# hpc4cmb/flacarray

Hardware: AMD Instinct MI355X
Metric: Msamples/s encode+decode, 4096ch x 1Msamp int32 (higher is better)
Workload: dtype int32

## Files before the change

### flacarray_amd/csrc/encode_fused.hpp

```cpp
#pragma once
#include "encode_kernels.hpp"
#include "quantize_kernels.hpp"

namespace fa {

constexpr int kFSmpWords = 65 * 32;
#ifndef FA_F_SCANW
#define FA_F_SCANW 4
#endif
#ifndef FA_F_RING
#define FA_F_RING 1024
#endif
constexpr int kFRingWords = FA_F_RING;
constexpr int kFRingMask = kFRingWords - 1;
constexpr int kFRingBlocks = kFRingWords / 64;
constexpr int kFRowBlocks = 12;
static_assert(kFRingBlocks - kFRowBlocks - 1 >= 1, "the ring must hold the longest row and a partial block beside what waits to be flushed");
constexpr int kFWaveWords = kFSmpWords + kFRingWords + 4 + 16;
constexpr int kFWaves = 4;
constexpr int kFCrcSlice = 1024;
constexpr int kFCrcXpow = 520;
#ifndef FA_F_SLEEP
#define FA_F_SLEEP 8
#endif
#ifndef FA_F_WBATCH
#define FA_F_WBATCH 4
#endif
#ifndef FA_F_CEIL
#define FA_F_CEIL 1
#endif
#ifndef FA_F_BFLY_N
#define FA_F_BFLY_N 1
#endif
#ifndef FA_F_SHLEV
#define FA_F_SHLEV 1
#endif
#ifndef FA_F_SHLEV_MAXMLO
#define FA_F_SHLEV_MAXMLO 12
#endif
#ifndef FA_F_SHPOLL
#define FA_F_SHPOLL 256
#endif
#ifndef FA_F_SHSLEEP
#define FA_F_SHSLEEP 4
#endif
#ifndef FA_F_PARKN
#define FA_F_PARKN 32
#endif
#ifndef FA_F_PARKBLK
#define FA_F_PARKBLK 1
#endif
#ifndef FA_F_PARK
#define FA_F_PARK 1
#endif
#ifndef FA_F_WAVES
#define FA_F_WAVES 3
#endif
constexpr uint32_t kLbSpinLimit = 1u << 22;

struct FusedArgs {
    const int32_t* data;
    const float* f_offsets;
    const float* f_gains;
    int64_t n_stream, stream_size, nframes, total_frames;
    int32_t max_lpc_order, max_porder, precision, pmax_full;
    int32_t tail_bs;
    double escale_full;
    const float* win;
    const uint4* hdr;
    uint8_t* blob;
    int64_t capacity;
    int64_t hb;
    uint32_t* frame_bytes;
    int64_t* frame_abs;
    FrameInfo* info;
    uint32_t* ticket;
    uint32_t* size_pub;
    unsigned long long* off_pub;
    int64_t* total;
    int* err;
    const uint16_t* crc_tab;
    unsigned long long* stamps;
    int64_t* starts;
    int64_t* nbytes;
};

__device__ __forceinline__ int fsmp_unit(int c1, int u) { return 32 * c1 + 4 * (u ^ (c1 & 7)); }
__device__ __forceinline__ int fsmp_idx(int s) {
    const int c1 = (s >> 5) + 1;
    return fsmp_unit(c1, (s >> 2) & 7) + (s & 3);
}

__device__ __forceinline__ int lane_id_opaque() {
    int l;
    asm volatile("v_mbcnt_lo_u32_b32 %0, -1, 0\n\tv_mbcnt_hi_u32_b32 %0, -1, %0" : "=v"(l));
    return l;
}
__device__ __forceinline__ int rice_fold(int r) { return (int)(((uint32_t)r << 1) ^ (uint32_t)(r >> 31)); }
__device__ __forceinline__ int dpp_wave_shr1(int old, int v) { return __builtin_amdgcn_update_dpp(old, v, 0x138, 0xF, 0xF, false); }

__device__ __forceinline__ uint16_t crc16_mulmod(uint16_t a, uint16_t b) {
    uint32_t r = 0;
#pragma unroll
    for (int i = 15; i >= 0; --i) {
        r = (r << 1) ^ ((r & 0x8000u) ? 0x18005u : 0u);
        if ((b >> i) & 1) r ^= a;
    }
    return (uint16_t)r;
}

template <typename T>
__device__ __forceinline__ T lb_load(const T* p) { return __hip_atomic_load(p, __ATOMIC_RELAXED, __HIP_MEMORY_SCOPE_AGENT); }

struct SplitRiceSearch {
    int pred_order, pmax, lane;
    uint32_t TA, TB, S, n, pb, SC, best;
    int M, p, k, bpo, kb;
    bool slot;
    __device__ __forceinline__ void start(uint32_t ta, uint32_t tb, int pred_order_, int pmax_, int lane_) {
        pred_order = pred_order_; pmax = pmax_; lane = lane_;
        TA = wave_incl_scan_u32(ta);
        TB = wave_incl_scan_u32(tb);
    }
    __device__ __forceinline__ void gather() {
        M = (2 << pmax) - 1;
        const int Lp = M - lane;
        slot = (Lp >= 1);
        const int po = slot ? (31 - __clz(Lp)) : 0;
        p = lane - (M + 1 - (2 << po));
        const uint32_t psz = 4096u >> po;
        const int cpp = 128 >> po;
        const bool inB = (po > 0) && (p >= (1 << (po - 1)));
        const int ph = inB ? (p - (1 << (po - 1))) : p;
        int hi_l = (po == 0) ? 63 : ((ph + 1) * cpp - 1);
        int lo_l = (po == 0) ? -1 : (ph * cpp - 1);
        hi_l &= 63;
        const int lo_c = lo_l < 0 ? 0 : (lo_l & 63);
        const uint32_t ah = (uint32_t)__builtin_amdgcn_ds_bpermute(hi_l << 2, (int)TA);
        const uint32_t bh = (uint32_t)__builtin_amdgcn_ds_bpermute(hi_l << 2, (int)TB);
        const uint32_t al = (uint32_t)__builtin_amdgcn_ds_bpermute(lo_c << 2, (int)TA);
        const uint32_t bl = (uint32_t)__builtin_amdgcn_ds_bpermute(lo_c << 2, (int)TB);
        uint32_t s;
        if (po == 0) s = ah + bh;
        else s = (inB ? bh : ah) - ((lo_l >= 0) ? (inB ? bl : al) : 0u);
        S = slot ? s : 0u;
        n = psz - ((p == 0) ? (uint32_t)pred_order : 0u);
        n = slot ? n : 1u;
    }
    __device__ __forceinline__ void params() {
        const uint32_t fpd = 0x40000u / n;
        const uint32_t m1 = S - 1;
// ... 188 lines not shown
                }
            } else {
                double* mbv = reinterpret_cast<double*>(wscr + 224);
                if (sub < MLO) mbv[sub] = mybits;
                lds_fence();
#pragma unroll
                for (int o = 0; o < MLO; ++o) {
                    const double b = mbv[o];
                    if (o < usable && b < bestb) { bestb = b; bi = o; }
                }
            }
            wlo = bi + 1;
        }
        if (fbps <= 17) {
            const int limp = 32 - fbps - ilog2_u64((uint64_t)wlo);
            if (wprec > limp) wprec = limp;
        }
        wsh = 0;
#pragma unroll
        for (int j = 0; j < MLO; ++j) wq[j] = 0;
        wok = 0;
        if (wprec >= 2) wok = (quantize_coefs_t<MLO>(coef + (wlo - 1) * MLO, wlo, wprec, wq, &wsh) == 0) ? 1 : 0;
    };
    auto shlev_announce = [&](bool cand, int fbps, const double* ac) __attribute__((always_inline)) {
        const int ln = lane_id_opaque();
        if (ln == 0) {
            if (cand) {
#pragma unroll
                for (int j = 0; j <= MLO; ++j) lev_in[wave][j] = ac[j];
            }
            lev_bps[wave] = cand ? fbps : -1;
        }
        lds_fence();
        uint32_t before = 0;
        if (ln == 0) before = __hip_atomic_fetch_add(&lev_cnt, 1u, __ATOMIC_RELAXED, __HIP_MEMORY_SCOPE_WORKGROUP);
        lds_fence();
        if ((uint32_t)__builtin_amdgcn_readfirstlane((int)before) != (uint32_t)(kFWaves - 1)) return;
        const int fr = ln >> 4, sub = ln & 15;
        const int fbps_w = lev_bps[fr];
        double acw[MLO + 1];
#pragma unroll
        for (int j = 0; j <= MLO; ++j) acw[j] = lev_in[fr][j];
        if (fbps_w < 0) {
            acw[0] = 1.0;
#pragma unroll
            for (int j = 1; j <= MLO; ++j) acw[j] = 0.0;
        }
        int wok, wlo, wprec, wsh;
        int32_t wq[MLO];
        lpc_solve(std::integral_constant<int, 16>{}, acw, fbps_w, scr + 256 * fr, sub, wok, wlo, wprec, wsh, wq);
        if (sub == 0) {
            lev_out[fr][0] = wok; lev_out[fr][1] = wlo; lev_out[fr][2] = wprec; lev_out[fr][3] = wsh;
#pragma unroll
            for (int j = 0; j < MLO; ++j) lev_out[fr][4 + j] = wq[j];
        }
        lds_fence();
        if (sub == 0) __hip_atomic_store(&lev_rdy[fr], 1u, __ATOMIC_RELAXED, __HIP_MEMORY_SCOPE_WORKGROUP);
        lds_fence();
    };
    if constexpr (SHLEV) {
        bool mine = g < a.total_frames;
        if (mine && a.tail_bs != kMaxBlock) mine = ((uint32_t)g % (uint32_t)a.nframes) != (uint32_t)(a.nframes - 1);
        if (__builtin_expect(!mine, 0)) {
            shlev_announce(false, 0, nullptr);
            return;
        }
    }
    if (g >= a.total_frames) return;

    const int64_t s = (int64_t)((uint32_t)g / (uint32_t)a.nframes);
    const int64_t f = g - s * a.nframes;
    if (f == a.nframes - 1 && a.tail_bs != kMaxBlock) return;
    const int32_t* src = a.data + (s * a.stream_size + f * (int64_t)bs);
    float q_off = 0.0f, q_gain = 0.0f;
    if constexpr (F32IN) { q_off = a.f_offsets[s]; q_gain = a.f_gains[s]; }
    auto load_row = [&](int j) __attribute__((always_inline)) {
        const int4 v = reinterpret_cast<const int4*>(src)[64 * j + lane];
        if constexpr (F32IN)
            return make_int4(quantise_f32(__int_as_float(v.x), q_off, q_gain), quantise_f32(__int_as_float(v.y), q_off, q_gain),
                             quantise_f32(__int_as_float(v.z), q_off, q_gain), quantise_f32(__int_as_float(v.w), q_off, q_gain));
        else
            return v;
    };
    const float* win = a.win;
    const uint4 fhe = a.hdr[f];
    const uint32_t fh_bits = 32u + ((fhe.w >> 8) & 0xFFu) + ((fhe.w >> 16) & 0xFFu) + (fhe.w >> 24) + 8u;

#define FA_IMAGE_ADDRS                                                                  \
    const int ln_ = lane_id_opaque();                                                   \
    const int K = fsmp_unit(ln_ + 1, 0);                                                \
    const int rowbase = fsmp_unit((ln_ >> 3) + 1, ln_ & 7);                             \
    const int hist7 = fsmp_unit(ln_, 7), hist6 = fsmp_unit(ln_, 6), hist5 = fsmp_unit(ln_, 5); \
    (void)K; (void)rowbase; (void)hist7; (void)hist6; (void)hist5
    constexpr int tailA7 = 32 * 64 + 4 * (7 ^ (64 & 7)), tailA6 = 32 * 64 + 4 * (6 ^ (64 & 7)), tailA5 = 32 * 64 + 4 * (5 ^ (64 & 7));

    FA_STAMP_INIT;
#ifdef FA_TIMELINE
    const uint32_t tl_start_ = (uint32_t)__builtin_amdgcn_s_memrealtime();
#endif
    int4 Bv[8];
    uint32_t orv = 0;
    int mn, mx;
    {
        FA_IMAGE_ADDRS;
        int4 hi[8], lo[8];
#pragma unroll
        for (int j = 0; j < 8; ++j) hi[j] = load_row(8 + j);
#pragma unroll
        for (int j = 0; j < 8; ++j) lo[j] = load_row(j);
        if (lane < 32) smp[lane] = 0;
        mn = hi[0].x;
        mx = hi[0].x;
#pragma unroll
        for (int j = 0; j < 8; ++j) {
            orv |= (uint32_t)(hi[j].x | hi[j].y | hi[j].z | hi[j].w);
            mn = min(min(mn, hi[j].x), hi[j].y);
            mn = min(min(mn, hi[j].z), hi[j].w);
            mx = max(max(mx, hi[j].x), hi[j].y);
            mx = max(max(mx, hi[j].z), hi[j].w);
            *reinterpret_cast<int4*>(&smp[rowbase + 256 * j]) = hi[j];
        }
#pragma unroll
        for (int t = 0; t < 8; ++t) Bv[t] = *reinterpret_cast<const int4*>(&smp[K ^ (4 * t)]);
#pragma unroll
        for (int j = 0; j < 8; ++j) {
            orv |= (uint32_t)(lo[j].x | lo[j].y | lo[j].z | lo[j].w);
            mn = min(min(mn, lo[j].x), lo[j].y);
            mn = min(min(mn, lo[j].z), lo[j].w);
            mx = max(max(mx, lo[j].x), lo[j].y);
            mx = max(max(mx, lo[j].z), lo[j].w);
            *reinterpret_cast<int4*>(&smp[rowbase + 256 * j]) = lo[j];
        }
    }
    mn = wave_min_i32(mn);
    mx = wave_max_i32(mx);
    const bool is_const = (mn == mx);
    orv = wave_or_u32(orv);
    const int wasted = orv ? (__ffs((int)orv) - 1) : 0;
    const int bps = 32 - wasted;
    if (__builtin_expect(wasted != 0, 0)) {
        FA_IMAGE_ADDRS;
#pragma unroll
        for (int t = 0; t < 8; ++t) {
            Bv[t].x >>= wasted; Bv[t].y >>= wasted; Bv[t].z >>= wasted; Bv[t].w >>= wasted;
            int4* p = reinterpret_cast<int4*>(&smp[K ^ (4 * t)]);
            int4 v = *p;
            v.x >>= wasted; v.y >>= wasted; v.z >>= wasted; v.w >>= wasted;
            *p = v;
        }
        mn >>= wasted;
        mx >>= wasted;
    }
    const bool narrow = (mn >= -(1 << 24)) && (mx < (1 << 24));
    lds_fence();

    FA_STAMP(0);
    const uint64_t verbatim_bits = 8 + (uint64_t)wasted + (uint64_t)bs * (uint64_t)bps;
    int type = 1;
    int order = 0, porder = 0, shift = 0, precision = 0;
    int kbest = 0;
    bool img_is_residual = false;
    bool win_small_l = false, win_small_f = false;
    int fo = -1;
    int32_t qkeep[MLO];
#pragma unroll
    for (int j = 0; j < MLO; ++j) qkeep[j] = 0;
    const int pmax_geo = a.pmax_full;
    auto pmax_for = [&](int pred_order) __attribute__((always_inline)) {
        int pm = pmax_geo;
        while (pm > 0 && (bs >> pm) <= pred_order) pm--;
        return pm;
    };

    auto hist_b = [&](const int4& own, const int4& tail) __attribute__((always_inline)) {
        int4 h;
        h.x = dpp_wave_shr1(tail.x, own.x);
        h.y = dpp_wave_shr1(tail.y, own.y);
        h.z = dpp_wave_shr1(tail.z, own.z);
        h.w = dpp_wave_shr1(tail.w, own.w);
        return h;
    };

    uint64_t best_bits = verbatim_bits;
    bool lpc_cand = false;
    double autoc[MLO + 1];
    uint64_t fixA = 0, fixB = 0, est_fix = 0;
    int po_fix = 0, k_fix = 0, pmax_fix = 0;
    bool fuse_search = false;
    auto apply_fixed = [&]() __attribute__((always_inline)) {
        if (est_fix < best_bits) {
            best_bits = est_fix;
            type = 2;
            order = fo;
            porder = po_fix;
            kbest = k_fix;
        }
    };
    auto fixed_analysis = [&]() __attribute__((always_inline)) {
        double tot0 = 0.0, tot1 = 0.0, tot2 = 0.0, tot3 = 0.0, tot4 = 0.0;
        double mx0 = 0.0, mx1 = 0.0, mx2 = 0.0, mx3 = 0.0, mx4 = 0.0;
        uint64_t hA0 = 0, hA1 = 0, hA2 = 0, hA3 = 0, hA4 = 0;
        double dA0 = 0.0, dA1 = 0.0, dA2 = 0.0, dA3 = 0.0, dA4 = 0.0;
        if (__builtin_expect(narrow, 1)) {
            FA_IMAGE_ADDRS;
            const uint32_t BIAS = 0x80000000u;
            uint32_t s0 = 0, s1 = 0, s2 = 0, s3 = 0, s4 = 0;
            int p1, pe1, pe2, pe3;
            auto seed = [&](const int4& hh) __attribute__((always_inline)) {
                p1 = hh.w;
                pe1 = hh.w - hh.z;
                pe2 = pe1 - (hh.z - hh.y);
                pe3 = pe2 - ((hh.z - hh.y) - (hh.y - hh.x));
            };
            auto group = [&](auto mask_tag, const int4& xv, int gi0) __attribute__((always_inline)) {
                constexpr bool MASK = decltype(mask_tag)::value;
                const int xs[4] = {xv.x, xv.y, xv.z, xv.w};
#pragma unroll
                for (int e = 0; e < 4; ++e) {
                    const int x = xs[e];
                    const int e1 = x - p1, e2 = e1 - pe1, e3 = e2 - pe2;
                    const uint32_t xb = (uint32_t)x ^ BIAS;
                    const uint32_t n0 = sad_u32(xb, BIAS, s0);
                    const uint32_t n1 = sad_u32(xb, (uint32_t)p1 ^ BIAS, s1);
                    const uint32_t n2 = sad_u32((uint32_t)e1 ^ BIAS, (uint32_t)pe1 ^ BIAS, s2);
                    const uint32_t n3 = sad_u32((uint32_t)e2 ^ BIAS, (uint32_t)pe2 ^ BIAS, s3);
                    const uint32_t n4 = sad_u32((uint32_t)e3 ^ BIAS, (uint32_t)pe3 ^ BIAS, s4);
                    if constexpr (MASK) {
                        const int gi = gi0 + e;
                        s0 = n0;
                        s1 = (gi >= 1) ? n1 : s1;
                        s2 = (gi >= 2) ? n2 : s2;
                        s3 = (gi >= 3) ? n3 : s3;
                        s4 = (gi >= 4) ? n4 : s4;
                    } else {
                        s0 = n0; s1 = n1; s2 = n2; s3 = n3; s4 = n4;
                    }
                    p1 = x; pe1 = e1; pe2 = e2; pe3 = e3;
                }
            };
            uint64_t a0 = 0, a1 = 0, a2 = 0, a3 = 0, a4 = 0;
            auto fold = [&]() __attribute__((always_inline)) {
                a0 += s0; a1 += s1; a2 += s2; a3 += s3; a4 += s4;
                s0 = s1 = s2 = s3 = s4 = 0;
            };
            seed(*reinterpret_cast<const int4*>(&smp[hist7]));
            group(std::true_type{}, *reinterpret_cast<const int4*>(&smp[K]), 32 * lane);
#pragma unroll
            for (int t = 1; t < 4; ++t) group(std::false_type{}, *reinterpret_cast<const int4*>(&smp[K ^ (4 * t)]), 0);
            fold();
#pragma unroll
            for (int t = 4; t < 8; ++t) group(std::false_type{}, *reinterpret_cast<const int4*>(&smp[K ^ (4 * t)]), 0);
            fold();
            hA0 = a0; hA1 = a1; hA2 = a2; hA3 = a3; hA4 = a4;
            seed(hist_b(Bv[7], *reinterpret_cast<const int4*>(&smp[tailA7])));
#pragma unroll
            for (int t = 0; t < 4; ++t) group(std::false_type{}, Bv[t], 0);
            fold();
#pragma unroll
            for (int t = 4; t < 8; ++t) group(std::false_type{}, Bv[t], 0);
            fold();
            tot0 = (double)a0; tot1 = (double)a1; tot2 = (double)a2; tot3 = (double)a3; tot4 = (double)a4;
        } else {
            FA_IMAGE_ADDRS;
            double p1, pe1, pe2, pe3;
            auto seed = [&](const int4& h) __attribute__((always_inline)) {
                p1 = (double)h.w;
                pe1 = (double)h.w - (double)h.z;
                const double e1b = (double)h.z - (double)h.y;
                pe2 = pe1 - e1b;
                const double e2b = e1b - ((double)h.y - (double)h.x);
                pe3 = pe2 - e2b;
            };
            auto group = [&](const int4& xv, int gi0) __attribute__((always_inline)) {
                const int xs[4] = {xv.x, xv.y, xv.z, xv.w};
#pragma unroll
                for (int e = 0; e < 4; ++e) {
                    const int gi = gi0 + e;
                    const double xd = (double)xs[e];
                    const double e1 = xd - p1;
                    const double e2 = e1 - pe1;
                    const double e3 = e2 - pe2;
                    const double e4 = e3 - pe3;
                    const double a0 = fa_fabs(xd);
                    const double a1 = (gi >= 1) ? fa_fabs(e1) : 0.0;
                    const double a2 = (gi >= 2) ? fa_fabs(e2) : 0.0;
                    const double a3 = (gi >= 3) ? fa_fabs(e3) : 0.0;
                    const double a4 = (gi >= 4) ? fa_fabs(e4) : 0.0;
                    tot0 += a0; tot1 += a1; tot2 += a2; tot3 += a3; tot4 += a4;
                    mx0 = __builtin_fmax(mx0, a0);
                    mx1 = __builtin_fmax(mx1, a1);
                    mx2 = __builtin_fmax(mx2, a2);
                    mx3 = __builtin_fmax(mx3, a3);
                    mx4 = __builtin_fmax(mx4, a4);
                    p1 = xd; pe1 = e1; pe2 = e2; pe3 = e3;
                }
            };
            seed(*reinterpret_cast<const int4*>(&smp[hist7]));
#pragma unroll 1
            for (int t = 0; t < 8; ++t) group(*reinterpret_cast<const int4*>(&smp[K ^ (4 * t)]), 32 * lane + 4 * t);
            dA0 = tot0; dA1 = tot1; dA2 = tot2; dA3 = tot3; dA4 = tot4;
            seed(hist_b(Bv[7], *reinterpret_cast<const int4*>(&smp[tailA7])));
#pragma unroll
            for (int t = 0; t < 8; ++t) group(Bv[t], 4096);
        }
        FA_STAMP(1);
        {
            double tsum[5] = {tot0, tot1, tot2, tot3, tot4};
            wave_sum_butterfly_n<5>(tsum);
            const double T0 = tsum[0], T1 = tsum[1], T2 = tsum[2], T3 = tsum[3], T4 = tsum[4];
            double M0 = 0.0, M1 = 0.0, M2 = 0.0, M3 = 0.0, M4 = 0.0;
            if (!narrow) {
                M0 = wave_max_f64(mx0); M1 = wave_max_f64(mx1); M2 = wave_max_f64(mx2); M3 = wave_max_f64(mx3);
                M4 = wave_max_f64(mx4);
            }
            const double lim = 2147483647.0;
            double smallest = 1.8446744073709552e19;
            if (M0 <= lim && T0 < smallest) { fo = 0; smallest = T0; }
            if (M1 <= lim && T1 < smallest) { fo = 1; smallest = T1; }
            if (M2 <= lim && T2 < smallest) { fo = 2; smallest = T2; }
            if (M3 <= lim && T3 < smallest) { fo = 3; smallest = T3; }
            if (M4 <= lim && T4 < smallest) { fo = 4; smallest = T4; }
        }
        if (narrow) {
            const uint64_t tA = (fo == 0) ? hA0 : (fo == 1) ? hA1 : (fo == 2) ? hA2 : (fo == 3) ? hA3 : hA4;
            const double tt = (fo == 0) ? tot0 : (fo == 1) ? tot1 : (fo == 2) ? tot2 : (fo == 3) ? tot3 : tot4;
            fixA = tA;
            fixB = (uint64_t)tt - tA;
        } else {
            const double tA = (fo == 0) ? dA0 : (fo == 1) ? dA1 : (fo == 2) ? dA2 : (fo == 3) ? dA3 : dA4;
            const double tt = (fo == 0) ? tot0 : (fo == 1) ? tot1 : (fo == 2) ? tot2 : (fo == 3) ? tot3 : tot4;
            fixA = (uint64_t)tA;
            fixB = (uint64_t)(tt - tA);
        }
        pmax_fix = pmax_for(fo < 0 ? 0 : fo);
        const bool small_fix = __all((fixA < (1u << 24)) && (fixB < (1u << 24)));
        win_small_f = small_fix;
        fuse_search = !SHLEV && fo >= 0 && pmax_fix <= 5 && a.max_lpc_order > 0 && small_fix;
        if (__builtin_expect(fo >= 0 && !fuse_search, SHLEV ? 1 : 0)) {
            uint64_t rb;
            if (pmax_fix <= 5 && small_fix) {
                SplitRiceSearch fs;
                fs.start((uint32_t)fixA, (uint32_t)fixB, fo, pmax_fix, lane);
                fs.gather(); fs.params(); fs.totals();
#pragma unroll
                for (int o = 5; o >= 0; --o) fs.order(o);
                po_fix = fs.bpo; k_fix = fs.kb; rb = fs.best;
            } else {
                rb = split_rice_search_slow(fixA, fixB, fo, pmax_fix, lane, &po_fix, &k_fix);
            }
            est_fix = 8 + (uint64_t)wasted + (uint64_t)fo * (uint64_t)bps + rb;
            apply_fixed();
        }
        FA_STAMP(2);
    };

    if (__builtin_expect(is_const, 0)) {
        type = 0;
    } else {
        if constexpr (!SHLEV) fixed_analysis();
        if (__builtin_expect(a.max_lpc_order > 0, 1)) {
            FA_IMAGE_ADDRS;
            double acc[MLO + 1];
#pragma unroll
            for (int j = 0; j <= MLO; ++j) acc[j] = 0.0;
            SplitRiceSearch fs;
            if (fuse_search) fs.start((uint32_t)fixA, (uint32_t)fixB, fo, pmax_fix, lane);
            double hist[MLO];
            struct WinV { double w[4]; };
            auto load_win = [&](int i0) __attribute__((always_inline)) {
                const float4 f = *reinterpret_cast<const float4*>(win + i0);
                WinV v;
                v.w[0] = (double)f.x; v.w[1] = (double)f.y; v.w[2] = (double)f.z; v.w[3] = (double)f.w;
                return v;
            };
            auto lag_group = [&](const int4& xv, const WinV& wv) __attribute__((always_inline)) {
                const int xs[4] = {xv.x, xv.y, xv.z, xv.w};
#pragma unroll
                for (int e = 0; e < 4; ++e) {
                    const double d = (double)xs[e] * wv.w[e];
                    acc[0] = __builtin_fma(d, d, acc[0]);
#pragma unroll
                    for (int j = 0; j < MLO; ++j) acc[j + 1] = __builtin_fma(d, hist[j], acc[j + 1]);
#pragma unroll
                    for (int j = MLO - 1; j > 0; --j) hist[j] = hist[j - 1];
                    hist[0] = d;
                }
            };
            auto search_stage = [&](int tt) __attribute__((always_inline)) {
                if (!fuse_search) return;
                if (tt == 1) fs.gather();
                if (tt == 3) fs.params();
                if (tt == 5) fs.totals();
                if (tt >= 7 && tt <= 12) fs.order(12 - tt);
            };
#if FA_F_PARK
            {
                int4* const pk = reinterpret_cast<int4*>(ring) + lane;
#pragma unroll
                for (int t = 0; t < 4; ++t) pk[64 * t] = Bv[4 + t];
            }
#endif
            {
                const int g0 = 32 * lane;
                const int4 h7 = *reinterpret_cast<const int4*>(&smp[hist7]), h6 = *reinterpret_cast<const int4*>(&smp[hist6]);
                const int4 h5 = *reinterpret_cast<const int4*>(&smp[hist5]);
                const int hs[12] = {h7.w, h7.z, h7.y, h7.x, h6.w, h6.z, h6.y, h6.x, h5.w, h5.z, h5.y, h5.x};
#pragma unroll
                for (int j = 0; j < MLO; ++j) {
                    const float wh = (g0 - 1 - j >= 0) ? win[g0 - 1 - j] : 0.0f;
                    hist[j] = (double)hs[j] * (double)wh;
                }
#pragma unroll
                for (int tb = 0; tb < 8; tb += FA_F_WBATCH) {
                    WinV wv[FA_F_WBATCH];
#pragma unroll
                    for (int t = 0; t < FA_F_WBATCH; ++t) wv[t] = load_win(g0 + 4 * (tb + t));
#pragma unroll
                    for (int t = 0; t < FA_F_WBATCH; ++t) {
                        lag_group(*reinterpret_cast<const int4*>(&smp[K ^ (4 * (tb + t))]), wv[t]);
                        search_stage(tb + t);
                    }
                    __builtin_amdgcn_sched_barrier(0);
                }
            }
#if FA_F_PARK
            {
                uint32_t pin = 16u * (uint32_t)lane;
                asm volatile("" : "+v"(pin) : "v"(__double2loint(acc[MLO])));
                const int4* const pk = reinterpret_cast<const int4*>(reinterpret_cast<const char*>(ring) + pin);
#pragma unroll
                for (int t = 0; t < 4; ++t) Bv[4 + t] = pk[64 * t];
            }
#endif
            {
                const int g0 = 2048 + 32 * lane;
                const int4 h7 = hist_b(Bv[7], *reinterpret_cast<const int4*>(&smp[tailA7]));
                const int4 h6 = hist_b(Bv[6], *reinterpret_cast<const int4*>(&smp[tailA6]));
                int4 h5 = make_int4(0, 0, 0, 0);
                if constexpr (MLO > 8) h5 = hist_b(Bv[5], *reinterpret_cast<const int4*>(&smp[tailA5]));
                const int hs[12] = {h7.w, h7.z, h7.y, h7.x, h6.w, h6.z, h6.y, h6.x, h5.w, h5.z, h5.y, h5.x};
#pragma unroll
                for (int j = 0; j < MLO; ++j) hist[j] = (double)hs[j] * (double)win[g0 - 1 - j];
#pragma unroll
                for (int tb = 0; tb < 8; tb += FA_F_WBATCH) {
                    WinV wv[FA_F_WBATCH];
#pragma unroll
                    for (int t = 0; t < FA_F_WBATCH; ++t) wv[t] = load_win(g0 + 4 * (tb + t));
#pragma unroll
                    for (int t = 0; t < FA_F_WBATCH; ++t) {
                        lag_group(Bv[tb + t], wv[t]);
                        search_stage(8 + tb + t);
                    }
                    __builtin_amdgcn_sched_barrier(0);
                }
            }
            FA_STAMP(4);
            if (fuse_search) {
                po_fix = fs.bpo;
                k_fix = fs.kb;
                est_fix = 8 + (uint64_t)wasted + (uint64_t)fo * (uint64_t)bps + (uint64_t)fs.best;
                apply_fixed();
            }
#if FA_F_BFLY_N
#pragma unroll
            for (int j = 0; j <= MLO; ++j) autoc[j] = acc[j];
            wave_sum_butterfly_n<MLO + 1>(autoc);
#else
#pragma unroll
            for (int j = 0; j <= MLO; ++j) autoc[j] = wave_sum_butterfly(acc[j]);
#endif
            lpc_cand = (autoc[0] != 0.0);
        }
    }

    FA_STAMP(5);
    int ok = 0, lo = 0, prec = a.precision, sh = 0;
    int32_t qreg[MLO];
#pragma unroll
    for (int j = 0; j < MLO; ++j) qreg[j] = 0;
    if constexpr (SHLEV) {
        shlev_announce(lpc_cand, bps, autoc);
        FA_STAMP(6);
        if (!is_const) fixed_analysis();
        if (lpc_cand) {
#ifdef FA_STAMPS
            const unsigned long long tw0_ = fa_memtime();
#endif
            uint32_t up = 0, polls = 0;
            for (;;) {
                up = (uint32_t)__builtin_amdgcn_readfirstlane((int)__hip_atomic_load(&lev_rdy[wave], __ATOMIC_RELAXED, __HIP_MEMORY_SCOPE_WORKGROUP));
                if (up != 0 || ++polls > (uint32_t)FA_F_SHPOLL) break;
                __builtin_amdgcn_s_sleep(FA_F_SHSLEEP);
            }
// ... 62 lines not shown
                const double r = xd - pred;
#endif
                if constexpr (MASK) {
                    const bool v = (gi0 + e >= lo);
                    tl += v ? fa_fabs(r) : 0.0;
                    rs[e] = v ? fold_f64(r) : xs[e];
                } else {
                    tl += fa_fabs(r);
                    rs[e] = fold_f64(r);
                }
#pragma unroll
                for (int j = MLO - 1; j > 0; --j) hx[j] = hx[j - 1];
                hx[0] = xd;
            }
            return make_int4(rs[0], rs[1], rs[2], rs[3]);
        };
        constexpr int kWarmGroups = (MLO + 3) / 4;
        {
            const int hs[12] = {a7.w, a7.z, a7.y, a7.x, a6.w, a6.z, a6.y, a6.x, a5.w, a5.z, a5.y, a5.x};
#pragma unroll
            for (int j = 0; j < MLO; ++j) hx[j] = (double)hs[j];
#pragma unroll
            for (int t = 0; t < 8; ++t) {
                int4* px = reinterpret_cast<int4*>(&smp[K ^ (4 * t)]);
                if (t < kWarmGroups) *px = res_group(std::true_type{}, *px, 32 * lane + 4 * t, tlA);
                else *px = res_group(std::false_type{}, *px, 0, tlA);
            }
        }
        {
            const int hs[12] = {b7.w, b7.z, b7.y, b7.x, b6.w, b6.z, b6.y, b6.x, b5.w, b5.z, b5.y, b5.x};
#pragma unroll
            for (int j = 0; j < MLO; ++j) hx[j] = (double)hs[j];
#pragma unroll
            for (int t = 0; t < 8; ++t) Bv[t] = res_group(std::false_type{}, Bv[t], 0, tlB);
        }
        FA_STAMP(7);
        img_is_residual = true;
        const int pmax = pmax_for(lo);
        int po_l = 0, k_l = 0;
        uint64_t rbits;
        const bool small_l = __all((tlA < 16777216.0) && (tlB < 16777216.0));
        bool lpc_in_range = true;
        if (__builtin_expect(!small_l, 0)) {
            bool hit = false;
#pragma unroll 1
            for (int t = 0; t < 8; ++t) {
                const int4 ra = *reinterpret_cast<const int4*>(&smp[K ^ (4 * t)]);
                const int ras[4] = {ra.x, ra.y, ra.z, ra.w};
#pragma unroll
                for (int e = 0; e < 4; ++e) hit = hit || ((32 * lane + 4 * t + e >= lo) && (uint32_t)ras[e] == 0xffffffffu);
            }
#pragma unroll
            for (int t = 0; t < 8; ++t)
                hit = hit || (uint32_t)Bv[t].x == 0xffffffffu || (uint32_t)Bv[t].y == 0xffffffffu || (uint32_t)Bv[t].z == 0xffffffffu ||
                      (uint32_t)Bv[t].w == 0xffffffffu;
            lpc_in_range = !__any(hit);
        }
        win_small_l = small_l;
        if (pmax <= 5 && small_l) {
            SplitRiceSearch ls;
            ls.start((uint32_t)tlA, (uint32_t)tlB, lo, pmax, lane);
            ls.gather(); ls.params(); ls.totals();
#pragma unroll
            for (int o = 5; o >= 0; --o) ls.order(o);
            po_l = ls.bpo; k_l = ls.kb; rbits = ls.best;
        } else {
            rbits = split_rice_search_slow((uint64_t)tlA, (uint64_t)tlB, lo, pmax, lane, &po_l, &k_l);
        }
        if (lpc_in_range) {
            const uint64_t est = 8 + (uint64_t)wasted + 4 + 5 + (uint64_t)lo * (uint64_t)(prec + bps) + rbits;
            if (est < best_bits) {
                best_bits = est;
                type = 3;
                order = lo;
                porder = po_l;
                kbest = k_l;
                shift = sh;
                precision = prec;
#pragma unroll
                for (int j = 0; j < MLO; ++j) qkeep[j] = qreg[j];
            }
        }
    }
    lds_fence();

    FA_STAMP(8);
    const int lane_w = lane_id_opaque();
    auto reload_image = [&](auto fold_tag) __attribute__((always_inline)) {
        constexpr bool FOLD = decltype(fold_tag)::value;
        FA_IMAGE_ADDRS;
#pragma unroll 1
        for (int half = 1; half >= 0; --half) {
#pragma unroll
            for (int j = 0; j < 8; ++j) {
                int4 v = load_row(8 * half + j);
                v.x >>= wasted; v.y >>= wasted; v.z >>= wasted; v.w >>= wasted;
                if constexpr (FOLD) { v.x = rice_fold(v.x); v.y = rice_fold(v.y); v.z = rice_fold(v.z); v.w = rice_fold(v.w); }
                *reinterpret_cast<int4*>(&smp[rowbase + 256 * j]) = v;
            }
            if (half == 1) {
#pragma unroll
                for (int t = 0; t < 8; ++t) Bv[t] = *reinterpret_cast<const int4*>(&smp[K ^ (4 * t)]);
            }
        }
        lds_fence();
    };
    if (__builtin_expect(type == 2 && order == 0, 0)) {
        if (img_is_residual) {
            reload_image(std::true_type{});
        } else {
            FA_IMAGE_ADDRS;
#pragma unroll
            for (int t = 0; t < 8; ++t) {
                int4* px = reinterpret_cast<int4*>(&smp[K ^ (4 * t)]);
                int4 v = *px;
                v.x = rice_fold(v.x); v.y = rice_fold(v.y); v.z = rice_fold(v.z); v.w = rice_fold(v.w);
                *px = v;
                Bv[t].x = rice_fold(Bv[t].x); Bv[t].y = rice_fold(Bv[t].y); Bv[t].z = rice_fold(Bv[t].z); Bv[t].w = rice_fold(Bv[t].w);
            }
            lds_fence();
        }
        img_is_residual = true;
    } else if (__builtin_expect(type == 2, 0)) {
        if (img_is_residual) {
            reload_image(std::false_type{});
            img_is_residual = false;
        }
        {
            FA_IMAGE_ADDRS;
            const int4 ha = *reinterpret_cast<const int4*>(&smp[hist7]);
            const int4 hb2 = hist_b(Bv[7], *reinterpret_cast<const int4*>(&smp[tailA7]));
            lds_fence();
            int64_t x1, x2, x3, x4;
            auto fgroup = [&](const int4& xv, int gi0) __attribute__((always_inline)) {
                const int xs[4] = {xv.x, xv.y, xv.z, xv.w};
                int rs[4];
#pragma unroll
                for (int e = 0; e < 4; ++e) {
                    const int64_t x0 = xs[e];
                    int64_t r;
                    if (order == 0) r = x0;
                    else if (order == 1) r = x0 - x1;
                    else if (order == 2) r = x0 - 2 * x1 + x2;
                    else if (order == 3) r = x0 - 3 * x1 + 3 * x2 - x3;
                    else r = x0 - 4 * x1 + 6 * x2 - 4 * x3 + x4;
                    rs[e] = (gi0 + e >= order) ? rice_fold((int)r) : xs[e];
                    x4 = x3; x3 = x2; x2 = x1; x1 = x0;
                }
                return make_int4(rs[0], rs[1], rs[2], rs[3]);
            };
            x1 = ha.w; x2 = ha.z; x3 = ha.y; x4 = ha.x;
#pragma unroll 1
            for (int t = 0; t < 8; ++t) {
                int4* px = reinterpret_cast<int4*>(&smp[K ^ (4 * t)]);
                *px = fgroup(*px, 32 * lane_w + 4 * t);
            }
            x1 = hb2.w; x2 = hb2.z; x3 = hb2.y; x4 = hb2.x;
#pragma unroll
            for (int t = 0; t < 8; ++t) Bv[t] = fgroup(Bv[t], 4096);
            img_is_residual = true;
        }
        lds_fence();
    }

    bool rice2 = false;
    if (type >= 2) rice2 = __any((lane_w < (1 << porder)) && (kbest >= 15));
// ... 587 lines not shown
```

### flacarray_amd/csrc/flacarray_hip.hip

```cpp
#include <hip/hip_runtime.h>

#include <cmath>
#include <cstdio>
#include <cstdlib>
#include <cstring>
#include <algorithm>
#include <atomic>
#include <condition_variable>
#include <functional>
#include <map>
#include <memory>
#include <mutex>
#include <new>
#include <thread>
#include <vector>

#include <sys/mman.h>
#include <time.h>
#include <unistd.h>

#include "../../include/flacarray_hip.h"
#include "decode_kernels.hpp"
#ifndef FA_SPLIT_UNITS
#define FA_HAVE_K5_LAUNCHERS 1
#endif
#include "encode_kernels.hpp"
#include "encode_fused.hpp"
#include "encode_placed.hpp"
#include "decode_latency.hpp"
#include "quantize_kernels.hpp"
#include "verify_kernels.hpp"
#include "std_kernels.hpp"
#include "splice_kernels.hpp"
#include "md5_kernels.hpp"
#include "reduce_kernels.hpp"
#include "histogram_kernels.hpp"
#include "scrub_kernels.hpp"
#include "reindex_kernels.hpp"
#include "window_kernels.hpp"
#include "join_kernels.hpp"

namespace {

using namespace fa;

#define FA_HIP_TRY(expr)                                                                          \
    do {                                                                                          \
        hipError_t e_ = (expr);                                                                   \
        if (e_ != hipSuccess) {                                                                   \
            std::fprintf(stderr, "flacarray_hip: %s failed: %s\n", #expr, hipGetErrorString(e_)); \
            return FA_ERROR_DEVICE;                                                               \
        }                                                                                         \
    } while (0)

constexpr int kProfPairs = 6;
constexpr int kScratchSlots = 23;
struct DeviceState {
    std::recursive_mutex api_mu;
    std::map<int, float*> windows;
    uint16_t* crc_tab = nullptr;
    uint16_t* crc_tab_fused = nullptr;
    void* scratch[kScratchSlots] = {};
    size_t scratch_bytes[kScratchSlots] = {};
    uint64_t scratch_epoch = 1;
    std::vector<uint4> h_hdr;
    int64_t c_nf = -1;
    int c_B = 0, c_tail = 0, c_nch = 0;
    void* c_dp = nullptr;
    uint64_t c_epoch = 0;
    bool stamps_zeroed = false;
    int64_t std_plan_key[2] = {-1, -1};
    uint64_t std_plan_epoch = 0;
    hipStream_t feed_stream = nullptr;
    void* pin = nullptr;
    void* pin_dev = nullptr;
    bool pin_tried = false;
    hipStream_t verify_stream = nullptr;
    hipEvent_t verify_ev[2] = {nullptr, nullptr};
    bool verify_tried = false;
    hipEvent_t ev[2 * kProfPairs];
    bool ev_ready = false;
    bool ev_set[kProfPairs] = {false, false, false, false, false, false};
};
std::mutex g_mu;
std::map<int, std::unique_ptr<DeviceState>> g_dev;
std::atomic<bool> g_prof{false};
std::atomic<bool> g_verify{false};
std::atomic<bool> g_encode_verify{false};
std::atomic<bool> g_encode_md5{false};

DeviceState* dev_state() {
    int d = 0;
    if (hipGetDevice(&d) != hipSuccess) return nullptr;
    std::lock_guard<std::mutex> lk(g_mu);
    auto& p = g_dev[d];
    if (!p) p.reset(new DeviceState());
    return p.get();
}
#define FA_API_LOCK_OR(fail_stmt)      \
    DeviceState* ds_ = dev_state();    \
    if (!ds_) { fail_stmt; }           \
    std::lock_guard<std::recursive_mutex> api_lock_(ds_->api_mu)
#define FA_API_LOCK FA_API_LOCK_OR(return FA_ERROR_DEVICE)

[[noreturn]] void fatal_device(const char* fn, const char* what) {
    std::fprintf(stderr, "flacarray_hip: %s: %s failed (%s); this entry point has no error channel and no CPU fallback\n", fn, what,
                 hipGetErrorString(hipGetLastError()));
    std::abort();
}

void prof_begin(int k, hipStream_t st) {
    if (!g_prof) return;
    DeviceState* ds = dev_state();
    if (!ds) return;
    if (!ds->ev_ready) {
        for (auto& e : ds->ev) (void)hipEventCreate(&e);
        ds->ev_ready = true;
    }
    (void)hipEventRecord(ds->ev[2 * k], st);
}
void prof_end(int k, hipStream_t st) {
    if (!g_prof) return;
    DeviceState* ds = dev_state();
    if (!ds) return;
    (void)hipEventRecord(ds->ev[2 * k + 1], st);
    ds->ev_set[k] = true;
}

int get_scratch(int slot, size_t bytes, void** out) {
    DeviceState* st = dev_state();
    if (!st) return FA_ERROR_DEVICE;
    if (st->scratch_bytes[slot] < bytes) {
        if (st->scratch[slot]) (void)hipFree(st->scratch[slot]);
        st->scratch[slot] = nullptr;
        st->scratch_bytes[slot] = 0;
        st->scratch_epoch++;
        size_t want = bytes + (bytes >> 3) + 256;
        if (hipMalloc(&st->scratch[slot], want) != hipSuccess) {
            if (hipMalloc(&st->scratch[slot], bytes) != hipSuccess) return FA_ERROR_ALLOC | FA_ERROR_DEVICE;
            want = bytes;
        }
        st->scratch_bytes[slot] = want;
    }
    *out = st->scratch[slot];
    return FA_ERROR_NONE;
}

void tukey_window(int L, std::vector<float>& w) {
    w.assign((size_t)L, 1.0f);
    const int Np = (int)(0.25f * (float)L) - 1;
    if (Np > 0) {
        for (int n = 0; n <= Np; ++n) {
            w[(size_t)n] = (float)(0.5 - 0.5 * std::cos(3.14159265358979323846 * (double)n / (double)Np));
            w[(size_t)(L - Np - 1 + n)] = (float)(0.5 - 0.5 * std::cos(3.14159265358979323846 * (double)(n + Np) / (double)Np));
        }
    }
}

int get_window(int L, const float** out) {
    DeviceState* st = dev_state();
    if (!st) return FA_ERROR_DEVICE;
    auto it = st->windows.find(L);
    if (it == st->windows.end()) {
        std::vector<float> w;
        tukey_window(L, w);
        float* d = nullptr;
        FA_HIP_TRY(hipMalloc(&d, sizeof(float) * (size_t)(L + 16)));
        FA_HIP_TRY(hipMemset(d, 0, sizeof(float) * (size_t)(L + 16)));
        FA_HIP_TRY(hipMemcpy(d, w.data(), sizeof(float) * (size_t)L, hipMemcpyHostToDevice));
        it = st->windows.emplace(L, d).first;
    }
    *out = it->second;
    return FA_ERROR_NONE;
}

int get_crc_tab(const uint16_t** out) {
    DeviceState* st = dev_state();
    if (!st) return FA_ERROR_DEVICE;
    if (!st->crc_tab) {
        std::vector<uint16_t> t((size_t)kCrcTabWords);
        auto feed = [](uint16_t c, uint8_t v) { return crc16_byte(c, v); };
        for (int k = 0; k < 4; ++k)
            for (int v = 0; v < 256; ++v) {
                uint16_t c = 0;
                for (int b = 0; b < 4; ++b) c = feed(c, (uint8_t)(b == k ? v : 0));
                t[(size_t)(k * 256 + v)] = c;
            }
        for (int v = 0; v < 256; ++v) {
            uint16_t hi = (uint16_t)(v << 8), lo = (uint16_t)v;
            for (int b = 0; b < 256; ++b) { hi = feed(hi, 0); lo = feed(lo, 0); }
            t[(size_t)(1024 + v)] = hi;
            t[(size_t)(1280 + v)] = lo;
        }
        uint16_t xp = 1;
        for (int n = 0; n < 512; ++n) {
            t[(size_t)(1536 + n)] = xp;
            xp = feed(xp, 0);
        }
        uint16_t* d = nullptr;
        FA_HIP_TRY(hipMalloc(&d, sizeof(uint16_t) * (size_t)kCrcTabWords));
        FA_HIP_TRY(hipMemcpy(d, t.data(), sizeof(uint16_t) * (size_t)kCrcTabWords, hipMemcpyHostToDevice));
        st->crc_tab = d;
    }
    *out = st->crc_tab;
    return FA_ERROR_NONE;
}

int get_crc_tab_fused(const uint16_t** out) {
    DeviceState* st = dev_state();
    if (!st) return FA_ERROR_DEVICE;
    if (!st->crc_tab_fused) {
        std::vector<uint16_t> t((size_t)(kFCrcSlice + kFCrcXpow));
        auto mulx8 = [](uint16_t c) { return crc16_byte(c, 0); };
        auto mulmod = [](uint16_t a, uint16_t b) {
            uint32_t r = 0;
            for (int i = 15; i >= 0; --i) {
                r = (r << 1) ^ ((r & 0x8000u) ? 0x18005u : 0u);
                if ((b >> i) & 1) r ^= a;
            }
            return (uint16_t)r;
        };
        int ord = 0;
        for (uint16_t c = 1;;) { c = mulx8(c); ++ord; if (c == 1) break; }
        auto xpow8 = [&](long k) {
            k %= ord;
            if (k < 0) k += ord;
            uint16_t c = 1;
            for (long i = 0; i < k; ++i) c = mulx8(c);
            return c;
        };
        const uint16_t x2016 = xpow8(252);
        for (int k = 0; k < 4; ++k)
            for (int v = 0; v < 256; ++v) {
                uint16_t c = 0;
                for (int b = 0; b < 4; ++b) c = crc16_byte(c, (uint8_t)(b == k ? v : 0));
                t[(size_t)(k * 256 + v)] = mulmod(c, x2016);
            }
        {
            uint16_t c = xpow8(-255);
            for (int i = 0; i < kFCrcXpow; ++i) { t[(size_t)(kFCrcSlice + i)] = c; c = mulx8(c); }
        }
        uint16_t* d = nullptr;
        FA_HIP_TRY(hipMalloc(&d, sizeof(uint16_t) * t.size()));
        FA_HIP_TRY(hipMemcpy(d, t.data(), sizeof(uint16_t) * t.size(), hipMemcpyHostToDevice));
        st->crc_tab_fused = d;
    }
    *out = st->crc_tab_fused;
    return FA_ERROR_NONE;
}

inline size_t align_up(size_t v, size_t a) { return (v + a - 1) / a * a; }

struct FramePlan {
// ... 929 lines not shown
                          fp.slot_stride);
    prof_end(1, st);
    prof_end(3, st);
    FA_HIP_TRY(hipGetLastError());
    return FA_ERROR_NONE;
}

int fa_encode_i32_device_finish(int64_t n_stream, int64_t stream_size, uint32_t level, void* d_workspace,
                                const int64_t* d_starts, unsigned char* d_bytes, void* stream) {
    return encode_device_finish(1, n_stream, stream_size, level, d_workspace, d_starts, d_bytes, stream);
}

int fa_encode_i64_device_finish(int64_t n_stream, int64_t stream_size, uint32_t level, void* d_workspace,
                                const int64_t* d_starts, unsigned char* d_bytes, void* stream) {
    return encode_device_finish(2, n_stream, stream_size, level, d_workspace, d_starts, d_bytes, stream);
}

int fa_encode_single_pass_supported(int64_t n_stream, int64_t stream_size, uint32_t level) {
    FramePlan fp;
    return (make_frame_plan(n_stream, stream_size, level, 1, &fp) == FA_ERROR_NONE && !slots_forced()) ? 1 : 0;
}

static int64_t capacity_bytes_for(int64_t n_stream, int64_t stream_size, uint32_t level, int nch) {
    FramePlan fp;
    if (make_frame_plan(n_stream, stream_size, level, nch, &fp) != FA_ERROR_NONE) return -1;
    return fp.capacity;
}
int64_t fa_encode_capacity_bytes(int64_t n_stream, int64_t stream_size, uint32_t level) { return capacity_bytes_for(n_stream, stream_size, level, 1); }
int64_t fa_encode_capacity_bytes_i64(int64_t n_stream, int64_t stream_size, uint32_t level) { return capacity_bytes_for(n_stream, stream_size, level, 2); }

static int64_t single_pass_need(const FramePlan& fp) {
    int64_t need = (int64_t)placed_layout(fp).total;
    if (fused_geometry(fp)) need = std::max<int64_t>(need, (int64_t)fused_layout(fp).total);
    return need;
}
static int64_t single_pass_workspace_for(int64_t n_stream, int64_t stream_size, uint32_t level, int nch) {
    FramePlan fp;
    if (make_frame_plan(n_stream, stream_size, level, nch, &fp) != FA_ERROR_NONE) return -1;
    return slots_forced() ? (int64_t)slot_layout(fp).total : single_pass_need(fp);
}
int64_t fa_encode_single_pass_workspace_bytes(int64_t n_stream, int64_t stream_size, uint32_t level) {
    return single_pass_workspace_for(n_stream, stream_size, level, 1);
}
int64_t fa_encode_single_pass_workspace_bytes_i64(int64_t n_stream, int64_t stream_size, uint32_t level) {
    return single_pass_workspace_for(n_stream, stream_size, level, 2);
}

static int fused_encode_run(const FramePlan& fp, const void* d_data, bool f32, const float* d_quanta, float* d_offsets, float* d_gains,
                            void* d_workspace, int64_t workspace_bytes, unsigned char* d_bytes, int64_t capacity_bytes, int64_t* d_starts,
                            int64_t* d_nbytes, int64_t* h_total_bytes, int32_t* d_info, void* stream) {
    FA_API_LOCK;
    const FusedLayout pl = fused_layout(fp);
    const int64_t n_stream = fp.n_stream, stream_size = fp.stream_size;
    if (!d_workspace || workspace_bytes < single_pass_need(fp)) return FA_ERROR_ALLOC;
    if (!d_bytes || capacity_bytes < n_stream * fp.hb + 64) return FA_ERROR_ALLOC;
    hipStream_t st = reinterpret_cast<hipStream_t>(stream);
    char* ws = reinterpret_cast<char*>(d_workspace);
    prof_begin(3, st);
    int* d_nanflag = reinterpret_cast<int*>(ws + pl.pub.off_ticket + 12);
    FA_HIP_TRY(hipMemsetAsync(ws + pl.pub.off_zero, 0, pl.pub.zero_bytes, st));
    if (f32) {
        const int64_t cps = (stream_size + kRangeChunk - 1) / kRangeChunk;
        void* pp = nullptr;
        int rcp = get_scratch(10, (size_t)n_stream * (size_t)cps * 8 + 256, &pp);
        if (rcp) return rcp;
        float* pmin = reinterpret_cast<float*>(pp);
        float* pmax = pmin + n_stream * cps;
        prof_begin(5, st);
        hipLaunchKernelGGL(float32_range_kernel, dim3((unsigned)(n_stream * cps)), dim3(256), 0, st, reinterpret_cast<const float*>(d_data),
                           stream_size, cps, pmin, pmax, d_nanflag);
        hipLaunchKernelGGL(float32_params_kernel, dim3((unsigned)((n_stream + 255) / 256)), dim3(256), 0, st, pmin, pmax, n_stream, cps,
                           d_quanta, d_offsets, d_gains);
        prof_end(5, st);
    }
    FusedArgs a;
    std::memset(&a, 0, sizeof a);
    a.data = reinterpret_cast<const int32_t*>(d_data); a.f_offsets = d_offsets; a.f_gains = d_gains; a.n_stream = n_stream; a.stream_size = stream_size; a.nframes = fp.nf; a.total_frames = fp.F;
    a.max_lpc_order = fp.P.max_lpc_order; a.max_porder = fp.P.max_porder; a.precision = fp.P.qlp_precision;
    a.pmax_full = fp.pmax_full;
    a.escale_full = fp.escale_full;
    a.tail_bs = fp.tail_bs;
    const bool tails = (fp.tail_bs != kMaxBlock);
    int rc = get_window(kMaxBlock, &a.win);
    if (rc) return rc;
    rc = get_crc_tab_fused(&a.crc_tab);
    if (rc) return rc;
    rc = frame_header_table(ds_, fp, st, &a.hdr);
    if (rc) return rc;
    a.blob = d_bytes; a.capacity = capacity_bytes; a.hb = fp.hb;
    point_into_publish_block(pl.pub, ws, &a);
    a.info = reinterpret_cast<FrameInfo*>(d_info);
    a.stamps = stamps_scratch(ds_);
    if (tails) {
        EncodeArgs t;
        rc = fill_encode_args(fp, a.data, reinterpret_cast<uint8_t*>(ws + pl.off_tslots), a.frame_bytes, d_info, &t);
        if (rc) return rc;
        t.hdr = a.hdr;
        t.tail_only = 1;
        launch_encode_for(t, 1, n_stream, st);
        launch_fused_tail_publish(st, a.frame_bytes, a.size_pub, n_stream, fp.nf);
    }
    prof_begin(0, st);
    launch_fused_encode(st, a, f32);
    prof_end(0, st);
    PublishBack back = {0, 0, 0};
    rc = read_publish_back(a, st, &back);
    if (rc) return rc;
    if (tails) {
        uint32_t* tb = reinterpret_cast<uint32_t*>(ws + pl.off_tbytes);
        int64_t* toff = reinterpret_cast<int64_t*>(ws + pl.off_toff);
        int64_t* tzero = reinterpret_cast<int64_t*>(ws + pl.off_tzero);
        launch_fused_tail_prep(st, a.off_pub, a.frame_bytes, n_stream, fp.nf, a.frame_abs, tb, toff, tzero);
        const uint16_t* crc5 = nullptr;
        rc = get_crc_tab(&crc5);
        if (rc) return rc;
        int64_t nblk = (n_stream + 3) / 4;
        if (nblk > 32768) nblk = 32768;
        launch_compact_frames(st, nblk, reinterpret_cast<const uint8_t*>(ws + pl.off_tslots), tb, toff, tzero, 1, n_stream, crc5, d_bytes, kSlotBytes);
    }
    launch_fused_finish(st, d_bytes, a.frame_abs, a.frame_bytes, n_stream, fp.nf, stream_size, (int32_t)kMaxBlock, (int32_t)fp.tail_bs, 1, fp.hb,
                        d_starts, d_nbytes, a.total);
    prof_end(3, st);
    FA_HIP_TRY(hipGetLastError());
    *h_total_bytes = back.total;
    if (back.nan & 1) return FA_ERROR_NAN_INPUT;
    return FA_ERROR_NONE;
}


static bool placed_preferred(const FramePlan& fp) {
    int64_t below = (fp.tail_bs == kMaxBlock) ? kPlacedBelowFrames / 4 : kPlacedBelowFrames;
    if (const char* e = std::getenv("FLACARRAY_HIP_PLACED_BELOW")) below = std::atoll(e);
    return fp.F < below;
}

static int placed_encode_run(const FramePlan& fp, const int32_t* d_data, void* d_workspace, int64_t workspace_bytes, unsigned char* d_bytes,
                             int64_t capacity_bytes, int64_t* d_starts, int64_t* d_nbytes, int64_t* h_total_bytes, int32_t* d_info,
                             void* stream) {
    FA_API_LOCK;
    const PlacedLayout pl = placed_layout(fp);
    if (!d_workspace || workspace_bytes < single_pass_need(fp)) return FA_ERROR_ALLOC;
    if (!d_bytes || capacity_bytes < fp.n_stream * fp.hb + 64) return FA_ERROR_ALLOC;
    hipStream_t st = reinterpret_cast<hipStream_t>(stream);
    char* ws = reinterpret_cast<char*>(d_workspace);
    prof_begin(3, st);
    FA_HIP_TRY(hipMemsetAsync(ws + pl.pub.off_zero, 0, pl.pub.zero_bytes, st));
    EncodeArgs a;
    int rc = fill_encode_args(fp, d_data, reinterpret_cast<uint8_t*>(ws + pl.off_slots), reinterpret_cast<uint32_t*>(ws + pl.pub.off_fbytes), d_info, &a);
    if (rc) return rc;
    rc = frame_header_table(ds_, fp, st, &a.hdr);
    if (rc) return rc;
    FusedArgs p;
    std::memset(&p, 0, sizeof p);
    p.n_stream = fp.n_stream; p.stream_size = fp.stream_size; p.nframes = fp.nf; p.total_frames = fp.F;
    p.blob = d_bytes; p.capacity = capacity_bytes; p.hb = fp.hb;
    point_into_publish_block(pl.pub, ws, &p);
    p.info = a.info;
    rc = get_crc_tab(&p.crc_tab);
    if (rc) return rc;
    p.stamps = a.stamps = stamps_scratch(ds_);
    if (p.stamps) (void)hipMemsetAsync(p.stamps + 28, 0, 8, st);
    p.starts = d_starts;
    p.nbytes = d_nbytes;
    prof_begin(0, st);
    launch_encode_placed(st, a, p, fp.nch, placed_grid(fp.F));
    prof_end(0, st);
// ... 2124 lines not shown
```

Before: 216,100.

## Prune fixed-predictor rice search with lower bound and use double-precision window table

```diff
diff --git a/flacarray_amd/csrc/encode_fused.hpp b/flacarray_amd/csrc/encode_fused.hpp
--- a/flacarray_amd/csrc/encode_fused.hpp
+++ b/flacarray_amd/csrc/encode_fused.hpp
@@ -53,6 +53,9 @@
 #ifndef FA_F_PARK
 #define FA_F_PARK 1
 #endif
+#ifndef FA_F_WIND
+#define FA_F_WIND 1
+#endif
 #ifndef FA_F_WAVES
 #define FA_F_WAVES 3
 #endif
@@ -67,6 +70,7 @@
     int32_t tail_bs;
     double escale_full;
     const float* win;
+    const double* wind;
     const uint4* hdr;
     uint8_t* blob;
     int64_t capacity;
@@ -421,7 +425,11 @@
         else
             return v;
     };
+#if FA_F_WIND
+    const double* win = a.wind;
+#else
     const float* win = a.win;
+#endif
     const uint4 fhe = a.hdr[f];
     const uint32_t fh_bits = 32u + ((fhe.w >> 8) & 0xFFu) + ((fhe.w >> 16) & 0xFFu) + (fhe.w >> 24) + 8u;
 
@@ -534,6 +542,20 @@
             porder = po_fix;
             kbest = k_fix;
         }
+    };
+    auto fixed_search = [&](int ln) __attribute__((always_inline)) {
+        uint64_t rb;
+        if (pmax_fix <= 5 && win_small_f) {
+            SplitRiceSearch fs;
+            fs.start((uint32_t)fixA, (uint32_t)fixB, fo, pmax_fix, ln);
+            fs.gather(); fs.params(); fs.totals();
+#pragma unroll
+            for (int o = 5; o >= 0; --o) fs.order(o);
+            po_fix = fs.bpo; k_fix = fs.kb; rb = fs.best;
+        } else {
+            rb = split_rice_search_slow(fixA, fixB, fo, pmax_fix, ln, &po_fix, &k_fix);
+        }
+        return rb;
     };
     auto fixed_analysis = [&]() __attribute__((always_inline)) {
         double tot0 = 0.0, tot1 = 0.0, tot2 = 0.0, tot3 = 0.0, tot4 = 0.0;
@@ -674,23 +696,60 @@
         pmax_fix = pmax_for(fo < 0 ? 0 : fo);
         const bool small_fix = __all((fixA < (1u << 24)) && (fixB < (1u << 24)));
         win_small_f = small_fix;
-        fuse_search = !SHLEV && fo >= 0 && pmax_fix <= 5 && a.max_lpc_order > 0 && small_fix;
-        if (__builtin_expect(fo >= 0 && !fuse_search, SHLEV ? 1 : 0)) {
-            uint64_t rb;
-            if (pmax_fix <= 5 && small_fix) {
-                SplitRiceSearch fs;
-                fs.start((uint32_t)fixA, (uint32_t)fixB, fo, pmax_fix, lane);
-                fs.gather(); fs.params(); fs.totals();
-#pragma unroll
-                for (int o = 5; o >= 0; --o) fs.order(o);
-                po_fix = fs.bpo; k_fix = fs.kb; rb = fs.best;
-            } else {
-                rb = split_rice_search_slow(fixA, fixB, fo, pmax_fix, lane, &po_fix, &k_fix);
-            }
-            est_fix = 8 + (uint64_t)wasted + (uint64_t)fo * (uint64_t)bps + rb;
-            apply_fixed();
+        if constexpr (!SHLEV) {
+            fuse_search = fo >= 0 && pmax_fix <= 5 && a.max_lpc_order > 0 && small_fix;
+            if (__builtin_expect(fo >= 0 && !fuse_search, 0)) {
+                est_fix = 8 + (uint64_t)wasted + (uint64_t)fo * (uint64_t)bps + fixed_search(lane);
+                apply_fixed();
+            }
         }
         FA_STAMP(2);
+    };
+    auto resolve_fixed = [&]() __attribute__((always_inline)) {
+        if (fo < 0) return;
+        const uint64_t limit = best_bits + (type == 3 ? 1u : 0u);
+        const uint64_t base = 8 + (uint64_t)wasted + (uint64_t)fo * (uint64_t)bps;
+        const int ln = lane_id_opaque();
+        auto chunk_lb = [&](uint64_t S, uint32_t n) __attribute__((always_inline)) {
+            const int b = 64 - __clzll((long long)S);
+            const int k0 = b > 6 ? b - 6 : 0;
+            const uint64_t S2 = S << 1;
+            uint64_t m = (((uint32_t)(2 * k0 + 1) * n) >> 1) + (S2 >> k0);
+            m = min(m, (uint64_t)(((uint32_t)(2 * k0 + 3) * n) >> 1) + (S2 >> (k0 + 1)));
+            m = min(m, (uint64_t)(((uint32_t)(2 * k0 + 5) * n) >> 1) + (S2 >> (k0 + 2)));
+            return (uint32_t)m;
+        };
+        auto chunk_lb32 = [&](uint32_t S, uint32_t n) __attribute__((always_inline)) {
+            const int b = 32 - __clz((int)S);
+            const int k0 = b > 6 ? b - 6 : 0;
+            const uint32_t S2 = S << 1;
+            uint32_t m = (((uint32_t)(2 * k0 + 1) * n) >> 1) + (S2 >> k0);
+            m = min(m, (((uint32_t)(2 * k0 + 3) * n) >> 1) + (S2 >> (k0 + 1)));
+            m = min(m, (((uint32_t)(2 * k0 + 5) * n) >> 1) + (S2 >> (k0 + 2)));
+            return m;
+        };
+        const uint32_t nA = 32u - (ln == 0 ? (uint32_t)fo : 0u);
+        uint32_t lbl;
+        if (__builtin_expect(win_small_f, 1)) lbl = chunk_lb32((uint32_t)fixA, nA) + chunk_lb32((uint32_t)fixB, 32u);
+        else lbl = chunk_lb(fixA, nA) + chunk_lb(fixB, 32u);
+        const uint32_t LB = 9u + (uint32_t)__builtin_amdgcn_readlane((int)wave_incl_scan_u32(lbl), 63);
+#ifdef FA_STAMPS
+        if (ln == 0 && a.stamps && (blockIdx.x & 63) == 0) {
+            atomicAdd(&a.stamps[21], 1ULL);
+            atomicAdd(&a.stamps[22], base + LB >= limit ? 1ULL : 0ULL);
+            atomicAdd(&a.stamps[23], type == 3 ? 1ULL : 0ULL);
+            atomicAdd(&a.stamps[24], (type == 3 && base + LB >= limit) ? 1ULL : 0ULL);
+        }
+#endif
+        if (__builtin_expect(base + LB >= limit, 1)) return;
+        est_fix = base + fixed_search(ln);
+        if (est_fix < limit) {
+            best_bits = est_fix;
+            type = 2;
+            order = fo;
+            porder = po_fix;
+            kbest = k_fix;
+        }
     };
 
     if (__builtin_expect(is_const, 0)) {
@@ -707,9 +766,14 @@
             double hist[MLO];
             struct WinV { double w[4]; };
             auto load_win = [&](int i0) __attribute__((always_inline)) {
+                WinV v;
+#if FA_F_WIND
+                const double2 f0 = *reinterpret_cast<const double2*>(win + i0), f1 = *reinterpret_cast<const double2*>(win + i0 + 2);
+                v.w[0] = f0.x; v.w[1] = f0.y; v.w[2] = f1.x; v.w[3] = f1.y;
+#else
                 const float4 f = *reinterpret_cast<const float4*>(win + i0);
-                WinV v;
                 v.w[0] = (double)f.x; v.w[1] = (double)f.y; v.w[2] = (double)f.z; v.w[3] = (double)f.w;
+#endif
                 return v;
             };
             auto lag_group = [&](const int4& xv, const WinV& wv) __attribute__((always_inline)) {
@@ -746,8 +810,8 @@
                 const int hs[12] = {h7.w, h7.z, h7.y, h7.x, h6.w, h6.z, h6.y, h6.x, h5.w, h5.z, h5.y, h5.x};
 #pragma unroll
                 for (int j = 0; j < MLO; ++j) {
-                    const float wh = (g0 - 1 - j >= 0) ? win[g0 - 1 - j] : 0.0f;
-                    hist[j] = (double)hs[j] * (double)wh;
+                    const double wh = (g0 - 1 - j >= 0) ? (double)win[g0 - 1 - j] : 0.0;
+                    hist[j] = (double)hs[j] * wh;
                 }
 #pragma unroll
                 for (int tb = 0; tb < 8; tb += FA_F_WBATCH) {
@@ -976,6 +1040,7 @@
             }
         }
     }
+    if constexpr (SHLEV) resolve_fixed();
     lds_fence();
 
     FA_STAMP(8);
diff --git a/flacarray_amd/csrc/flacarray_hip.hip b/flacarray_amd/csrc/flacarray_hip.hip
--- a/flacarray_amd/csrc/flacarray_hip.hip
+++ b/flacarray_amd/csrc/flacarray_hip.hip
@@ -58,6 +58,7 @@
 struct DeviceState {
     std::recursive_mutex api_mu;
     std::map<int, float*> windows;
+    std::map<int, double*> windows_d;
     uint16_t* crc_tab = nullptr;
     uint16_t* crc_tab_fused = nullptr;
     void* scratch[kScratchSlots] = {};
@@ -169,6 +170,24 @@
         FA_HIP_TRY(hipMemset(d, 0, sizeof(float) * (size_t)(L + 16)));
         FA_HIP_TRY(hipMemcpy(d, w.data(), sizeof(float) * (size_t)L, hipMemcpyHostToDevice));
         it = st->windows.emplace(L, d).first;
+    }
+    *out = it->second;
+    return FA_ERROR_NONE;
+}
+
+int get_window_d(int L, const double** out) {
+    DeviceState* st = dev_state();
+    if (!st) return FA_ERROR_DEVICE;
+    auto it = st->windows_d.find(L);
+    if (it == st->windows_d.end()) {
+        std::vector<float> w;
+        tukey_window(L, w);
+        std::vector<double> wd(w.begin(), w.end());
+        double* d = nullptr;
+        FA_HIP_TRY(hipMalloc(&d, sizeof(double) * (size_t)(L + 16)));
+        FA_HIP_TRY(hipMemset(d, 0, sizeof(double) * (size_t)(L + 16)));
+        FA_HIP_TRY(hipMemcpy(d, wd.data(), sizeof(double) * (size_t)L, hipMemcpyHostToDevice));
+        it = st->windows_d.emplace(L, d).first;
     }
     *out = it->second;
     return FA_ERROR_NONE;
@@ -1264,6 +1283,8 @@
     a.tail_bs = fp.tail_bs;
     const bool tails = (fp.tail_bs != kMaxBlock);
     int rc = get_window(kMaxBlock, &a.win);
+    if (rc) return rc;
+    rc = get_window_d(kMaxBlock, &a.wind);
     if (rc) return rc;
     rc = get_crc_tab_fused(&a.crc_tab);
     if (rc) return rc;
```

New measurement: 217,600, median of 2. Within noise of the previous version (+0.7%).
